# tensorboy/pytorch_Realtime_Multi-Person_Pose_Estimation

Hardware: AMD Instinct MI355X
Metric: end-to-end persons-posed FPS at 368x368 (net+pafprocess) (higher is better)
Workload: dtype fp32; 1 GPU; rtpose VGG19 368x368 batch=32 synthetic images, single MI355X, fp32 (BASELINE.json configs[1]); per-GPU batch 32, one process per GPU; global_batch=32, weights=seeded He init (no checkpoint offline), decoder_input=synthetic scene + 1e-3 * net output (blend kernel timed), humans_per_batch=163, parallelism=single GPU

## Files before the change

pytorch_realtime_multi-person_pose_estimation_amd/csrc/conv_wino7.hip:

```cpp
#include <hip/hip_runtime.h>

#include <cstdlib>

#include "conv_desc.h"
#include "launchers.h"
#include "wino_common.h"

namespace rtpose {

namespace wino7 {

using namespace winoc;

constexpr int W7_PF = 4;

template <int FM>
struct WT;
template <>
struct WT<4> {
  static constexpr int NFQ = 10, NP = 4, NSETS = 5;
  __device__ static constexpr float kPts[4] = {1.f, 2.f, 0.5f, 1.5f};
  __device__ static constexpr float kBT[10][10] = {
      {2.25f, 0.f, -12.8125f, 0.f, 17.0625f, 0.f, -7.5f, 0.f, 1.f, 0.f},
      {0.f, -2.25f, -2.25f, 10.5625f, 10.5625f, -6.5f, -6.5f, 1.f, 1.f, 0.f},
      {0.f, 2.25f, -2.25f, -10.5625f, 10.5625f, 6.5f, -6.5f, -1.f, 1.f, 0.f},
      {0.f, -1.125f, -0.5625f, 6.125f, 3.0625f, -7.f, -3.5f, 2.f, 1.f, 0.f},
      {0.f, 1.125f, -0.5625f, -6.125f, 3.0625f, 7.f, -3.5f, -2.f, 1.f, 0.f},
      {0.f, -4.5f, -9.f, 7.625f, 15.25f, -3.625f, -7.25f, 0.5f, 1.f, 0.f},
      {0.f, 4.5f, -9.f, -7.625f, 15.25f, 3.625f, -7.25f, -0.5f, 1.f, 0.f},
      {0.f, -1.5f, -1.f, 7.875f, 5.25f, -7.875f, -5.25f, 1.5f, 1.f, 0.f},
      {0.f, 1.5f, -1.f, -7.875f, 5.25f, 7.875f, -5.25f, -1.5f, 1.f, 0.f},
      {0.f, 2.25f, 0.f, -12.8125f, 0.f, 17.0625f, 0.f, -7.5f, 0.f, 1.f},
  };
};
template <>
struct WT<6> {
  static constexpr int NFQ = 12, NP = 5, NSETS = 6;
  __device__ static constexpr float kPts[5] = {1.f, 2.f, 0.5f, 1.5f, 0.666666667f};
  __device__ static constexpr float kBT[12][12] = {
      {-1.f, 0.f, 7.94444444f, 0.f, -20.3958333f, 0.f, 20.3958333f, 0.f, -7.94444444f, 0.f, 1.f, 0.f},
      {0.f, 1.f, 1.f, -6.94444444f, -6.94444444f, 13.4513889f, 13.4513889f, -6.94444444f, -6.94444444f, 1.f, 1.f, 0.f},
      {0.f, -1.f, 1.f, 6.94444444f, -6.94444444f, -13.4513889f, 13.4513889f, 6.94444444f, -6.94444444f, -1.f, 1.f, 0.f},
      {0.f, 0.5f, 0.25f, -3.84722222f, -1.92361111f, 9.23611111f, 4.61805556f, -7.88888889f, -3.94444444f, 2.f, 1.f, 0.f},
      {0.f, -0.5f, 0.25f, 3.84722222f, -1.92361111f, -9.23611111f, 4.61805556f, 7.88888889f, -3.94444444f, -2.f, 1.f, 0.f},
      {0.f, 2.f, 4.f, -7.88888889f, -15.7777778f, 9.23611111f, 18.4722222f, -3.84722222f, -7.69444444f, 0.5f, 1.f, 0.f},
      {0.f, -2.f, 4.f, 7.88888889f, -15.7777778f, -9.23611111f, 18.4722222f, 3.84722222f, -7.69444444f, -0.5f, 1.f, 0.f},
      {0.f, 0.666666667f, 0.444444444f, -5.f, -3.33333333f, 11.375f, 7.58333333f, -8.54166667f, -5.69444444f, 1.5f, 1.f, 0.f},
      {0.f, -0.666666667f, 0.444444444f, 5.f, -3.33333333f, -11.375f, 7.58333333f, 8.54166667f, -5.69444444f, -1.5f, 1.f, 0.f},
      {0.f, 1.5f, 2.25f, -8.54166667f, -12.8125f, 11.375f, 17.0625f, -5.f, -7.5f, 0.666666667f, 1.f, 0.f},
      {0.f, -1.5f, 2.25f, 8.54166667f, -12.8125f, -11.375f, 17.0625f, 5.f, -7.5f, -0.666666667f, 1.f, 0.f},
      {0.f, -1.f, 0.f, 7.94444444f, 0.f, -20.3958333f, 0.f, 20.3958333f, 0.f, -7.94444444f, 0.f, 1.f},
  };
};

template <>
struct WT<8> {
  static constexpr int NFQ = 14, NP = 6, NSETS = 7;
  __device__ static constexpr float kPts[6] = {1.f, 2.f, 0.5f, 1.5f, 0.666666667f, 1.25f};
  __device__ static constexpr float kBT[14][14] = {
      {1.5625f, 0.f, -13.4131944f, 0.f, 39.812934f, 0.f, -52.2643229f, 0.f, 32.8090278f, 0.f, -9.50694444f, 0.f, 1.f, 0.f},
      {0.f, -1.5625f, -1.5625f, 11.8506944f, 11.8506944f, -27.9622396f, -27.9622396f, 24.3020833f, 24.3020833f, -8.50694444f, -8.50694444f, 1.f, 1.f, 0.f},
      {0.f, 1.5625f, -1.5625f, -11.8506944f, 11.8506944f, 27.9622396f, -27.9622396f, -24.3020833f, 24.3020833f, 8.50694444f, -8.50694444f, -1.f, 1.f, 0.f},
      {0.f, -0.78125f, -0.390625f, 6.51128472f, 3.25564236f, -18.2786458f, -9.13932292f, 21.5625f, 10.78125f, -11.0138889f, -5.50694444f, 2.f, 1.f, 0.f},
      {0.f, 0.78125f, -0.390625f, -6.51128472f, 3.25564236f, 18.2786458f, -9.13932292f, -21.5625f, 10.78125f, 11.0138889f, -5.50694444f, -2.f, 1.f, 0.f},
      {0.f, -3.125f, -6.25f, 14.3263889f, 28.6527778f, -22.3203125f, -44.640625f, 15.2473958f, 30.4947917f, -4.62847222f, -9.25694444f, 0.5f, 1.f, 0.f},
      {0.f, 3.125f, -6.25f, -14.3263889f, 28.6527778f, 22.3203125f, -44.640625f, -15.2473958f, 30.4947917f, 4.62847222f, -9.25694444f, -0.5f, 1.f, 0.f},
      {0.f, -1.04166667f, -0.694444444f, 8.47916667f, 5.65277778f, -22.7734375f, -15.1822917f, 24.7213542f, 16.4809028f, -10.8854167f, -7.25694444f, 1.5f, 1.f, 0.f},
      {0.f, 1.04166667f, -0.694444444f, -8.47916667f, 5.65277778f, 22.7734375f, -15.1822917f, -24.7213542f, 16.4809028f, 10.8854167f, -7.25694444f, -1.5f, 1.f, 0.f},
      {0.f, -2.34375f, -3.515625f, 14.8463542f, 22.2695312f, -26.3151042f, -39.4726562f, 19.1875f, 28.78125f, -6.04166667f, -9.0625f, 0.666666667f, 1.f, 0.f},
      {0.f, 2.34375f, -3.515625f, -14.8463542f, 22.2695312f, 26.3151042f, -39.4726562f, -19.1875f, 28.78125f, 6.04166667f, -9.0625f, -0.666666667f, 1.f, 0.f},
      {0.f, -1.25f, -1.f, 9.93055556f, 7.94444444f, -25.4947917f, -20.3958333f, 25.4947917f, 20.3958333f, -9.93055556f, -7.94444444f, 1.25f, 1.f, 0.f},
      {0.f, 1.25f, -1.f, -9.93055556f, 7.94444444f, 25.4947917f, -20.3958333f, -25.4947917f, 20.3958333f, 9.93055556f, -7.94444444f, -1.25f, 1.f, 0.f},
      {0.f, 1.5625f, 0.f, -13.4131944f, 0.f, 39.812934f, 0.f, -52.2643229f, 0.f, 32.8090278f, 0.f, -9.50694444f, 0.f, 1.f},
  };
};

#define RTPOSE_W7_POINTS {0.0, 1.0, -1.0, 2.0, -2.0, 0.5, -0.5, 1.5, -1.5, 2.0 / 3.0, -2.0 / 3.0, 1.25, -1.25}

struct Group {
  const float* in;
  const float* w;
  const float* bias;
  float* out;
  int in_cstride, in_choff, in_ws, in_hs, in_lead;
  int out_cstride, out_choff, out_ws, out_hs, out_lead;
  int cout, cout_pad;
  size_t in_bytes, w_bytes;
};

struct Args {
  Group g[2];
  int N, H, W;
  int GX, T;
  int TPI;
  int cin, relu;
  int RS;
  int VB;
  int mtiles, ntiles, ncombo, xcd_remap;
  int persist;
  float* scratch;
  int* flags;
  int* err;
};

__device__ float llvm_raw_buffer_load_f32(i32x4 rsrc, int voffset, int soffset, int aux) __asm(
    "llvm.amdgcn.raw.buffer.load.f32");

constexpr int CK = 8, CG = 2;

__host__ __device__ constexpr int row_stride(int gx, int nfq) {
  int rs = nfq * CG * gx;
  while ((rs & 15) != (gx & 15)) ++rs;
  return rs;
}
__host__ __device__ constexpr int strip_rows(int gx) { return (31 + gx - 1) / gx + 1 + 6; }

template <int NI, int FM>
struct Xform {
  using T = WT<FM>;
  static constexpr int NFQ = T::NFQ, NP = T::NP, NHI = NFQ - 7;
  i32x4 rin;
  unsigned voff[NI], vhi[NI][NHI], pxb;
  int vdst[NI], fstride;
  F4 d[NI][NFQ], eo[2];

  __device__ __forceinline__ void setup(const Group& g, int W, int GX, int RS, int R0, int nrows) {
    const int tid = threadIdx.x;
    const int nitems = nrows * GX * CG;
    const long qbase = (long)g.in_lead + (long)(R0 - 3) * g.in_ws - 3;
    const size_t o0 = (size_t)qbase * g.in_cstride + g.in_choff;
    rin = make_rsrc(g.in + o0, g.in_bytes - o0 * 4);
#pragma unroll
    for (int k = 0; k < NI; ++k) {
      const int i = min((tid & 255) + k * 256, nitems - 1);
      const int r = i / (GX * CG), rem = i - r * (GX * CG);
      const int cg = rem / GX, gx = rem - cg * GX;
      voff[k] = (unsigned)((((long)r * g.in_ws + FM * gx) * g.in_cstride + cg * 4) * 4);
      vdst[k] = r * RS + cg * GX + gx;
#pragma unroll
      for (int n = 7; n < NFQ; ++n) vhi[k][n - 7] = voff[k] + (unsigned)(min(n, W + 5 - FM * gx) * g.in_cstride * 4);
    }
    pxb = (unsigned)g.in_cstride * 4;
    fstride = CG * GX;
  }
  __device__ __forceinline__ void load_piece(int chunk, int k, int n) {
    const unsigned cb = (unsigned)chunk * (CK * 4);
    d[k][n] = n < 7 ? bload(rin, voff[k], cb + n * pxb) : bload(rin, vhi[k][n < 7 ? 0 : n - 7], cb);
  }
  __device__ __forceinline__ void tgroup(float4* vw, int k, int gidx) {
    if (gidx < NP) {
      const int row = 2 * gidx + 1;
#pragma unroll
      for (int odd = 0; odd < 2; ++odd) {
        const int n0 = odd ? 1 : 2;
        F4 s = mul4(T::kBT[row][n0], d[k][n0]);
#pragma unroll
        for (int t = 1; t < NP; ++t) s = fma4(T::kBT[row][n0 + 2 * t], d[k][n0 + 2 * t], s);
        eo[odd] = s;
      }
      vw[vdst[k] + row * fstride] = to_float4(add4(eo[0], eo[1]));
      vw[vdst[k] + (row + 1) * fstride] = to_float4(sub4(eo[0], eo[1]));
    } else {
      const int f = gidx == NP ? 0 : NFQ - 1, n0 = gidx == NP ? 0 : 1;
      F4 s = mul4(T::kBT[f][n0], d[k][n0]);
#pragma unroll
      for (int t = 1; t < NP + 1; ++t) s = fma4(T::kBT[f][n0 + 2 * t], d[k][n0 + 2 * t], s);
      vw[vdst[k] + f * fstride] = to_float4(s);
    }
  }
};

template <int NI, int GXT, int FM, int FS>
__device__ __forceinline__ void wino7_segment(const Args& A, float4* V4, const int mt, const int c, const int cb,
                                              const int ce, const int nch, const int slot) {
  using T = WT<FM>;
  constexpr int NFQ = T::NFQ, NP = T::NP;
  constexpr int NFW = NFQ / FS;
  static_assert(NFW % 2 == 0, "frequency pairs");
  constexpr int NSETS = FS == 2 ? 7 : (FM == 6 && NI == 2) ? 3 : T::NSETS;
  constexpr int NPS = 7 * NFW / 2;
  constexpr int PF = FS == 2 ? NSETS - 1 : (W7_PF < NSETS ? W7_PF : NSETS - 1);
  static_assert(NPS % NSETS == 0, "B register sets must rotate in step with the chunk");
  const int tid = threadIdx.x;
  const int lane = tid & 63;
  const int wv = __builtin_amdgcn_readfirstlane(tid >> 6);
  const int wn = FS == 2 ? (wv & 3) : wv, fh = FS == 2 ? (wv >> 2) : 0;
  const bool xf = wv < 4;
  auto my_group = [&](int gi) { return true || (gi & 1) == fh; };
  const int l31 = lane & 31, kh = lane >> 5;
  const int nt = c % A.ntiles, grp = c / A.ntiles;
  const Group g = grp ? A.g[1] : A.g[0];
  const int GX = GXT ? GXT : A.GX;
  const int RS = GXT ? row_stride(GXT, NFQ) : A.RS;
  const int VB = GXT ? strip_rows(GXT) * row_stride(GXT, NFQ) : A.VB;
  const int PI = A.H * GX;

  int t0, tlim;
  if (A.TPI) {
    const int n = mt / A.TPI;
    t0 = n * PI + (mt - n * A.TPI) * 32;
    tlim = (n + 1) * PI;
  } else {
    t0 = mt * 32;
    tlim = A.T;
  }
  int R0, nrows;
  {
    const int n0 = t0 / PI, y0 = (t0 - n0 * PI) / GX;
    const int t1 = min(t0 + 31, tlim - 1);
    const int n1 = t1 / PI, y1 = (t1 - n1 * PI) / GX;
    R0 = n0 * g.in_hs + y0;
    nrows = n1 * g.in_hs + y1 - R0 + 7;
  }
  Xform<NI, FM> X;
  X.setup(g, A.W, GX, RS, R0, nrows);
  const i32x4 rw = make_rsrc(g.w, g.w_bytes);
  auto load_piece = [&](int chunk, int k, int n) { X.load_piece(chunk, k, n); };
  auto tgroup = [&](float4* vw, int k, int gidx) { X.tgroup(vw, k, gidx); };

  int abase;
  {
    const int t = min(t0 + l31, tlim - 1);
    const int n = t / PI, r = t - n * PI;
    const int y = r / GX, gx = r - y * GX;
    abase = (n * g.in_hs + y - R0) * RS + kh * GX + gx + (fh * NFW) * CG * GX;
  }
  const int ncol = nt * 128 + wn * 32 + l31;
  floatx16 acc[NFW];
  float* sp = A.scratch + ((size_t)(slot * 4 + wn) * (NFQ * 16) + (size_t)fh * NFW * 16) * 64 + lane;
  if (FM == 8) {
    if (cb > 0) {
      if (tid == 0) {
        unsigned spins = 0;
        while (__hip_atomic_load(A.flags + slot, __ATOMIC_ACQUIRE, __HIP_MEMORY_SCOPE_AGENT) != 1) {
          __builtin_amdgcn_s_sleep(8);
          if (++spins > (1u << 22)) {
            __hip_atomic_fetch_or(A.err, 1, __ATOMIC_RELAXED, __HIP_MEMORY_SCOPE_AGENT);
            break;
          }
        }
      }
      __syncthreads();
      __builtin_amdgcn_fence(__ATOMIC_ACQUIRE, "agent");
    }
    const i32x4 rs = make_rsrc(sp - lane, cb > 0 ? (size_t)NFW * 16 * 64 * sizeof(float) : 0);
    const float b0 = g.bias[ncol];
#pragma unroll
    for (int f = 0; f < NFW; ++f)
#pragma unroll
      for (int r = 0; r < 16; ++r) {
        const float v = llvm_raw_buffer_load_f32(rs, lane * 4, (f * 16 + r) * 256, 0);
        acc[f][r] = (f == 1 && cb == 0) ? b0 : v;
      }
    if (cb > 0) {
      __syncthreads();
      if (tid == 0) __hip_atomic_store(A.flags + slot, 0, __ATOMIC_RELAXED, __HIP_MEMORY_SCOPE_AGENT);
    }
  } else if (cb == 0) {
#pragma unroll
    for (int f = 0; f < NFW; ++f)
#pragma unroll
      for (int r = 0; r < 16; ++r) acc[f][r] = 0.f;
    if (fh == 0) {
      const float b0 = g.bias[ncol];
#pragma unroll
      for (int r = 0; r < 16; ++r) acc[1][r] = b0;
    }
  } else {
    if (tid == 0) {
      unsigned spins = 0;
      while (__hip_atomic_load(A.flags + slot, __ATOMIC_ACQUIRE, __HIP_MEMORY_SCOPE_AGENT) != 1) {
        __builtin_amdgcn_s_sleep(8);
        if (++spins > (1u << 22)) {
          __hip_atomic_fetch_or(A.err, 1, __ATOMIC_RELAXED, __HIP_MEMORY_SCOPE_AGENT);
          break;
        }
      }
    }
    __syncthreads();
    __builtin_amdgcn_fence(__ATOMIC_ACQUIRE, "agent");
#pragma unroll
    for (int f = 0; f < NFW; ++f)
#pragma unroll
      for (int r = 0; r < 16; ++r) acc[f][r] = sp[(f * 16 + r) * 64];
    __syncthreads();
    if (tid == 0) __hip_atomic_store(A.flags + slot, 0, __ATOMIC_RELAXED, __HIP_MEMORY_SCOPE_AGENT);
  }
  const unsigned boff = (unsigned)((kh * g.cout_pad + ncol) * 16);
  const unsigned fstep = (unsigned)(CG * g.cout_pad * 16);
  unsigned wso = ((unsigned)cb * (7 * NFQ) + (unsigned)(fh * NFW)) * fstep;
  int bl = 0;
  auto bnext = [&](int& cnt) {
    wso += fstep;
    if (++cnt == NFW) {
      cnt = 0;
      if (FS > 1) wso += (unsigned)(NFQ - NFW) * fstep;
    }
  };
  float4 bs[NSETS][2];

  if (xf) {
#pragma unroll
    for (int k = 0; k < NI; ++k)
#pragma unroll
      for (int n = 0; n < NFQ; ++n) load_piece(cb, k, n);
#pragma unroll
    for (int k = 0; k < NI; ++k)
#pragma unroll
      for (int gi = 0; gi < NP + 2; ++gi)
        tgroup(V4, k, gi);
    const int c1 = min(cb + 1, ce - 1);
#pragma unroll
    for (int k = 0; k < NI; ++k)
#pragma unroll
      for (int n = 0; n < NFQ; ++n) load_piece(c1, k, n);
  }
#pragma unroll
  for (int s = 0; s < PF; ++s) {
    bs[s][0] = bload_f4(rw, boff, wso);
    bnext(bl);
    bs[s][1] = bload_f4(rw, boff, wso);
    bnext(bl);
  }
  __syncthreads();

#define RTPOSE_PIN()             \
  asm volatile("" ::: "memory"); \
  __builtin_amdgcn_sched_barrier(0)
  constexpr int NG = (NP + 2) * NI, GSTR = (NI == 1 && FS == 1) ? 2 : 1, LS = NG * GSTR;
  constexpr int LPS = 1, LSTEPS = (NFQ * NI + LPS - 1) / LPS;
  static_assert(LS + LSTEPS <= NPS, "transform work does not fit the steps of a chunk");
  float4 a[2][2];
  for (int chunk = cb; chunk < ce; ++chunk) {
    const float4* va = V4 + ((chunk - cb) & 1) * VB + abase;
    float4* vw = V4 + ((chunk - cb + 1) & 1) * VB;
    const int c2 = min(chunk + 2, ce - 1);
    a[0][0] = va[0];
    a[0][1] = va[CG * GX];
#pragma unroll
    for (int ps = 0; ps < NPS; ++ps) {
      const int fp = ps % (NFW / 2);
#pragma unroll
      for (int j = 0; j < 4; ++j) {
        {
          const float4 a0 = a[ps & 1][0], a1 = a[ps & 1][1], b0 = bs[ps % NSETS][0], b1 = bs[ps % NSETS][1];
          const float a0v[4] = {a0.x, a0.y, a0.z, a0.w}, a1v[4] = {a1.x, a1.y, a1.z, a1.w};
          const float b0v[4] = {b0.x, b0.y, b0.z, b0.w}, b1v[4] = {b1.x, b1.y, b1.z, b1.w};
          acc[2 * fp] = __builtin_amdgcn_mfma_f32_32x32x2f32(a0v[j], b0v[j], acc[2 * fp], 0, 0, 0);
          acc[2 * fp + 1] = __builtin_amdgcn_mfma_f32_32x32x2f32(a1v[j], b1v[j], acc[2 * fp + 1], 0, 0, 0);
        }
        RTPOSE_PIN();
        if (j < 2) {
          if (ps + 1 < NPS) {
            const int kyn = (ps + 1) / (NFW / 2), fn = 2 * ((ps + 1) % (NFW / 2)) + j;
            a[(ps + 1) & 1][j] = va[kyn * RS + fn * CG * GX];
          }
        } else {
          bs[(ps + PF) % NSETS][j - 2] = bload_f4(rw, boff, wso);
          bnext(bl);
        }
        if (j == 3 && xf) {
          if (ps % GSTR == 0 && ps / GSTR < NG) {
            if (xf && my_group((ps / GSTR) % (NP + 2))) tgroup(vw, (ps / GSTR) / (NP + 2), (ps / GSTR) % (NP + 2));
          } else if (ps >= LS && ps < LS + LSTEPS) {
#pragma unroll
            for (int q = 0; q < LPS; ++q) {
              const int l = LPS * (ps - LS) + q;
              if (l < NFQ * NI) load_piece(c2, l / NFQ, l % NFQ);
            }
          }
        }
        RTPOSE_PIN();
      }
    }
    __syncthreads();
  }
#undef RTPOSE_PIN

  if (ce < nch) {
#pragma unroll
    for (int f = 0; f < NFW; ++f)
#pragma unroll
      for (int r = 0; r < 16; ++r) sp[(f * 16 + r) * 64] = acc[f][r];
    __builtin_amdgcn_fence(__ATOMIC_RELEASE, "agent");
    __syncthreads();
    if (tid == 0) __hip_atomic_store(A.flags + slot, 1, __ATOMIC_RELEASE, __HIP_MEMORY_SCOPE_AGENT);
    return;
  }

  const bool col_ok = ncol < g.cout;
  float* out_base = g.out + g.out_choff + ncol;
  constexpr int R0E = 16 / FS;
  float* E = reinterpret_cast<float*>(V4);
  if (FS == 2) {
    float* ew = E + (size_t)((wn * 2 + fh) * NFW * 8) * 64 + lane;
#pragma unroll
    for (int f = 0; f < NFW; ++f)
#pragma unroll
      for (int rl = 0; rl < 8; ++rl) ew[(f * 8 + rl) * 64] = fh ? acc[f][rl] : acc[f][8 + rl];
    __syncthreads();
  }
  const float* er = E + (size_t)((wn * 2 + (1 - fh)) * NFW * 8) * 64 + lane;
  int tcur = t0 + (FS == 2 ? 16 * fh : 0) + 4 * kh;
  int sn = tcur / PI, sy, sx;
  {
    const int r = tcur - sn * PI;
    sy = r / GX;
    sx = r - sy * GX;
  }
#pragma unroll
  for (int rr = 0; rr < R0E; ++rr) {
    const int r = rr;
    float m[NFQ];
    if (FS == 2) {
#pragma unroll
      for (int f = 0; f < NFW; ++f) {
        const float own = fh ? acc[f][8 + rr] : acc[f][rr];
        const float oth = er[(f * 8 + rr) * 64];
        m[f] = fh ? oth : own;
        m[NFW + f] = fh ? own : oth;
      }
    } else {
#pragma unroll
      for (int f = 0; f < NFQ; ++f) m[f] = acc[f % NFW][rr];
    }
    float S[NP], D[NP];
#pragma unroll
    for (int p = 0; p < NP; ++p) {
      S[p] = m[2 * p + 1] + m[2 * p + 2];
      D[p] = m[2 * p + 1] - m[2 * p + 2];
    }
    float y[FM];
#pragma unroll
    for (int i = 0; i < FM; ++i) {
      float v = (i & 1) ? D[0] : S[0];
      float pw[NP];
#pragma unroll
      for (int p = 1; p < NP; ++p) {
        pw[p] = 1.f;
        for (int e = 0; e < i; ++e) pw[p] *= T::kPts[p];
        v = __builtin_fmaf(pw[p], (i & 1) ? D[p] : S[p], v);
      }
      if (i == 0) v += m[0];
      if (i == FM - 1) v += m[NFQ - 1];
      y[i] = v;
    }
    if (col_ok && tcur < tlim) {
      const size_t q = (size_t)g.out_lead + (size_t)(sn * g.out_hs + sy) * g.out_ws + FM * sx;
#pragma unroll
      for (int i = 0; i < FM; ++i) {
        const float v = A.relu ? fmaxf(y[i], 0.f) : y[i];
        if (FM * sx + i < A.W) out_base[(q + i) * g.out_cstride] = v;
      }
    }
    const int dstep = (r & 3) == 3 ? 5 : 1;
    tcur += dstep;
    sx += dstep;
    while (sx >= GX) {
      sx -= GX;
      if (++sy >= A.H) {
        sy = 0;
        ++sn;
      }
    }
  }
  if (FS == 2) __syncthreads();
}

template <int NI, int GXT, int FM, int FS>
__global__ __launch_bounds__(256 * FS, 1) void wino7_f32(const Args A) {
  extern __shared__ __attribute__((aligned(16))) float4 V4[];
  const int nch = A.cin / CK;
  long u0, u1;
  if (A.persist) {
    const long U = (long)A.mtiles * A.ncombo * nch, P = gridDim.x, p = blockIdx.x;
    u0 = p * U / P;
    u1 = (p + 1) * U / P;
  } else {
    const int bi = blockIdx.x;
    int mt, c;
    if (A.xcd_remap) {
      const int xcd = bi & 7, j = bi >> 3;
      c = j % A.ncombo;
      mt = (j / A.ncombo) * 8 + xcd;
    } else {
      mt = bi % A.mtiles;
      c = bi / A.mtiles;
    }
    if (mt >= A.mtiles) return;
    u0 = ((long)mt * A.ncombo + c) * nch;
    u1 = u0 + nch;
  }
  const int tf = (int)(u0 / nch), cbf = (int)(u0 - (long)tf * nch);
  const int tl = (int)((u1 - 1) / nch), cel = (int)(u1 - (long)tl * nch);
  const int nseg = tl - tf + 1;
  for (int i = 0; i < nseg; ++i) {
    int tile, cb = 0, ce = nch;
    const bool head_first = cel < nch && nseg > 1, tail_last = cbf > 0;
    if (head_first && i == 0) {
      tile = tl;
      ce = cel;
    } else if (tail_last && i == nseg - 1) {
      tile = tf;
      cb = cbf;
      if (tf == tl) ce = cel;
    } else {
      tile = tf + i - (head_first ? 1 : 0) + (tail_last ? 1 : 0);
      if (tile == tl) ce = cel;
    }
    const int mt = tile / A.ncombo, c = tile - mt * A.ncombo;
    wino7_segment<NI, GXT, FM, FS>(A, V4, mt, c, cb, ce, nch, cb > 0 ? (int)blockIdx.x - 1 : (int)blockIdx.x);
  }
}

template <int NI>
__global__ __launch_bounds__(256, 1) void wino7s_f32(const Args A) {
  constexpr int FM = 6;
  using T = WT<FM>;
  constexpr int NFQ = T::NFQ, NP = T::NP, FW = NFQ / 4;
  constexpr int NSETS = 7, PF = 3;
  extern __shared__ __attribute__((aligned(16))) float4 V4[];
  const int tid = threadIdx.x;
  const int lane = tid & 63;
  const int wv = __builtin_amdgcn_readfirstlane(tid >> 6);
  const int l31 = lane & 31, kh = lane >> 5;
  const int bi = blockIdx.x;
  const int c = bi % A.ncombo, mt = bi / A.ncombo;
  const int nt = c % A.ntiles, grp = c / A.ntiles;
  const Group g = grp ? A.g[1] : A.g[0];
  const int GX = A.GX, RS = A.RS, VB = A.VB;
  const int PI = A.H * GX;
  int t0, tlim;
  if (A.TPI) {
    const int n = mt / A.TPI;
    t0 = n * PI + (mt - n * A.TPI) * 32;
    tlim = (n + 1) * PI;
  } else {
    t0 = mt * 32;
    tlim = A.T;
  }
  int R0, nrows;
  {
    const int n0 = t0 / PI, y0 = (t0 - n0 * PI) / GX;
    const int t1 = min(t0 + 31, tlim - 1);
    const int n1 = t1 / PI, y1 = (t1 - n1 * PI) / GX;
    R0 = n0 * g.in_hs + y0;
    nrows = n1 * g.in_hs + y1 - R0 + 7;
  }
  Xform<NI, FM> X;
  X.setup(g, A.W, GX, RS, R0, nrows);
  const i32x4 rw = make_rsrc(g.w, g.w_bytes);

  int abase;
  {
    const int t = min(t0 + l31, tlim - 1);
    const int n = t / PI, r = t - n * PI;
    const int y = r / GX, gx = r - y * GX;
    abase = (n * g.in_hs + y - R0) * RS + kh * GX + gx + (wv * FW) * CG * GX;
  }
  const int ncol = nt * 32 + l31;
  floatx16 acc[FW];
#pragma unroll
  for (int f = 0; f < FW; ++f)
#pragma unroll
    for (int r = 0; r < 16; ++r) acc[f][r] = 0.f;
  if (wv == 0) {
    const float b0 = g.bias[ncol];
#pragma unroll
    for (int r = 0; r < 16; ++r) acc[1][r] = b0;
  }
  const unsigned boff = (unsigned)((kh * g.cout_pad + ncol) * 16);
  const unsigned fstep = (unsigned)(CG * g.cout_pad * 16);
  const unsigned kstep = (unsigned)NFQ * fstep;
  const int nchunks = A.cin / CK;
  unsigned wso = (unsigned)(wv * FW) * fstep;
  const unsigned wso_max = wso + (unsigned)(nchunks * 7 - 1) * kstep;
  float4 bs[NSETS][FW];

#pragma unroll
  for (int k = 0; k < NI; ++k)
#pragma unroll
    for (int n = 0; n < NFQ; ++n) X.load_piece(0, k, n);
#pragma unroll
  for (int k = 0; k < NI; ++k)
#pragma unroll
    for (int gi = 0; gi < NP + 2; ++gi) X.tgroup(V4, k, gi);
  {
    const int c1 = min(1, nchunks - 1);
#pragma unroll
    for (int k = 0; k < NI; ++k)
#pragma unroll
      for (int n = 0; n < NFQ; ++n) X.load_piece(c1, k, n);
  }
#pragma unroll
  for (int s = 0; s < PF; ++s) {
#pragma unroll
    for (int f = 0; f < FW; ++f) bs[s][f] = bload_f4(rw, boff, wso + f * fstep);
    wso = min(wso + kstep, wso_max);
  }
  __syncthreads();

#define RTPOSE_PIN()             \
  asm volatile("" ::: "memory"); \
  __builtin_amdgcn_sched_barrier(0)
  constexpr int NG = (NP + 2) * NI;
  static_assert(NG <= 8 * NI && NFQ <= 12 && NI <= 2, "transform work does not fit the slots of a chunk");
  float4 a[2][FW];
  for (int chunk = 0; chunk < nchunks; ++chunk) {
    const float4* va = V4 + (chunk & 1) * VB + abase;
    float4* vw = V4 + ((chunk + 1) & 1) * VB;
    const int c2 = min(chunk + 2, nchunks - 1);
#pragma unroll
    for (int f = 0; f < FW; ++f) a[0][f] = va[f * CG * GX];
#pragma unroll
    for (int ky = 0; ky < 7; ++ky) {
#pragma unroll
      for (int j = 0; j < 4; ++j) {
#pragma unroll
        for (int f = 0; f < FW; ++f) {
          const float4 av = a[ky & 1][f], bv = bs[ky % NSETS][f];
          const float avv[4] = {av.x, av.y, av.z, av.w}, bvv[4] = {bv.x, bv.y, bv.z, bv.w};
          acc[f] = __builtin_amdgcn_mfma_f32_32x32x2f32(avv[j], bvv[j], acc[f], 0, 0, 0);
        }
        RTPOSE_PIN();
        if (j == 0) {
          if (ky + 1 < 7) {
#pragma unroll
            for (int f = 0; f < FW; ++f) a[(ky + 1) & 1][f] = va[(ky + 1) * RS + f * CG * GX];
          }
        } else if (j == 1) {
#pragma unroll
          for (int f = 0; f < FW; ++f) bs[(ky + PF) % NSETS][f] = bload_f4(rw, boff, wso + f * fstep);
          wso = min(wso + kstep, wso_max);
        } else {
          const int slot = 2 * ky + (j - 2);
#pragma unroll
          for (int q = 0; q < NI; ++q) {
            if (ky < 4) {
              const int gq = slot * NI + q;
              if (gq < NG) X.tgroup(vw, gq / (NP + 2), gq % (NP + 2));
            } else {
#pragma unroll
              for (int h = 0; h < 2; ++h) {
                const int l = ((slot - 8) * NI + q) * 2 + h;
                if (l < NFQ * NI) X.load_piece(c2, l / NFQ, l % NFQ);
              }
            }
          }
        }
        RTPOSE_PIN();
      }
    }
    __syncthreads();
  }
#undef RTPOSE_PIN

  float* E = reinterpret_cast<float*>(V4);
#pragma unroll
  for (int f = 0; f < FW; ++f)
#pragma unroll
    for (int r = 0; r < 16; ++r) E[((wv * FW + f) * 16 + r) * 64 + lane] = acc[f][r];
  __syncthreads();
  const bool col_ok = ncol < g.cout;
  float* out_base = g.out + g.out_choff + ncol;
  int tcur = t0 + 8 * wv + 4 * kh;
  int sn = tcur / PI, sy, sx;
  {
    const int r = tcur - sn * PI;
    sy = r / GX;
    sx = r - sy * GX;
  }
#pragma unroll
  for (int rr = 0; rr < 4; ++rr) {
    const int r = 4 * wv + rr;
    float m[NFQ];
#pragma unroll
    for (int f = 0; f < NFQ; ++f) m[f] = E[(f * 16 + r) * 64 + lane];
    float S[NP], D[NP];
#pragma unroll
    for (int p = 0; p < NP; ++p) {
      S[p] = m[2 * p + 1] + m[2 * p + 2];
      D[p] = m[2 * p + 1] - m[2 * p + 2];
    }
    float y[FM];
#pragma unroll
    for (int i = 0; i < FM; ++i) {
      float v = (i & 1) ? D[0] : S[0];
      float pw[NP];
#pragma unroll
      for (int p = 1; p < NP; ++p) {
        pw[p] = 1.f;
        for (int e = 0; e < i; ++e) pw[p] *= T::kPts[p];
        v = __builtin_fmaf(pw[p], (i & 1) ? D[p] : S[p], v);
      }
      if (i == 0) v += m[0];
      if (i == FM - 1) v += m[NFQ - 1];
      y[i] = v;
    }
    if (col_ok && tcur < tlim) {
      const size_t q = (size_t)g.out_lead + (size_t)(sn * g.out_hs + sy) * g.out_ws + FM * sx;
#pragma unroll
      for (int i = 0; i < FM; ++i) {
        const float v = A.relu ? fmaxf(y[i], 0.f) : y[i];
        if (FM * sx + i < A.W) out_base[(q + i) * g.out_cstride] = v;
      }
    }
    ++tcur;
    if (++sx >= GX) {
      sx = 0;
      if (++sy >= A.H) {
        sy = 0;
        ++sn;
      }
    }
  }
}

__global__ void pack_wino7_kernel(const float* __restrict__ w, const float* __restrict__ bias, int cout,
                                  int cin_src, const int32_t* __restrict__ cin_map, int cin_packed, int coutp,
                                  int nfq, float* __restrict__ wp, float* __restrict__ bp) {
  const size_t total = (size_t)7 * nfq * cin_packed * coutp;
  const size_t i = (size_t)blockIdx.x * blockDim.x + threadIdx.x;
  if (i < (size_t)coutp) bp[i] = (i < (size_t)cout && bias) ? bias[i] : 0.f;
  if (i >= total) return;
  const int e = i & 3;
  size_t r = i >> 2;
  const int n = r % coutp;
  r /= coutp;
  const int cg = r % CG;
  r /= CG;
  const int f = r % nfq;
  r /= nfq;
  const int ky = r % 7;
  const int chunk = r / 7;
  const int c = chunk * CK + cg * 4 + e;
  const int src = cin_map ? cin_map[c] : (c < cin_src ? c : -1);
  float v = 0.f;
  if (n < cout && src >= 0 && src < cin_src) {
    const float* gw = w + (((size_t)n * cin_src + src) * 7 + ky) * 7;
    if (f == nfq - 1) {
      v = gw[6];
    } else {
      const double pts[13] = RTPOSE_W7_POINTS;
      double nf = 1.0;
      for (int l = 0; l < nfq - 1; ++l)
        if (l != f) nf *= pts[f] - pts[l];
      double s = 0.0, pw = 1.0;
      for (int kx = 0; kx < 7; ++kx) {
        s += pw * (double)gw[kx];
        pw *= pts[f];
      }
      v = (float)(s / nf);
    }
  }
  wp[i] = v;
}

int wino7_default_fm() {
  static int fm = 0;
  if (!fm) {
    const char* e = getenv("RTPOSE_WINOGRAD7_M");
    fm = (e && e[0] == '4') ? 4 : 6;
  }
  return fm;
}
static int resolve_fm(int fm) { return fm == 0 ? wino7_default_fm() : fm; }

struct Plan {
  int fm, nfq, gx, rs, nrows, ni, tpi, mtiles;
  long T;
  size_t lds;
};

static int make_plan(int N, int H, int W, int hs, int fm, Plan* p) {
  p->fm = fm;
  p->nfq = p->fm + 6;
  p->gx = ceil_div(W, p->fm);
  p->rs = row_stride(p->gx, p->nfq);
  p->T = (long)N * H * p->gx;
  if (p->T > 0x7fffffffL) return -1;
  const int pi = H * p->gx;
  p->tpi = pi >= 256 ? ceil_div(pi, 32) : 0;
  int nrows = 0;
  if (p->tpi) {
    nrows = strip_rows(p->gx) < H + 6 ? strip_rows(p->gx) : H + 6;
    p->mtiles = N * p->tpi;
  } else {
    for (long t0 = 0; t0 < p->T; t0 += 32) {
      const long t1 = t0 + 31 < p->T - 1 ? t0 + 31 : p->T - 1;
      const int n0 = (int)(t0 / pi), y0 = (int)((t0 - (long)n0 * pi) / p->gx);
      const int n1 = (int)(t1 / pi), y1 = (int)((t1 - (long)n1 * pi) / p->gx);
      const int rows = (n1 * hs + y1) - (n0 * hs + y0) + 7;
      if (rows > nrows) nrows = rows;
    }
    p->mtiles = (int)((p->T + 31) / 32);
  }
  p->nrows = nrows;
  p->ni = ceil_div(nrows * p->gx * CG, 256);
  p->lds = (size_t)2 * nrows * p->rs * 16;
  return 0;
}

template <int NI, int GXT, int FM, int FS = 1>
static int launch_inst(const Args& a, dim3 grid, size_t lds, hipStream_t s) {
  const size_t ex = FS == 2 ? (size_t)4 * 2 * (FM + 6) / 2 * 8 * 64 * sizeof(float) : 0;
  return launch_kernel<wino7_f32<NI, GXT, FM, FS>>(grid, dim3(256 * FS), lds > ex ? lds : ex, 160 * 1024, s, a);
}

template <int NI>
static int launch_small(const Args& a, dim3 grid, size_t lds, hipStream_t s) {
  return launch_kernel<wino7s_f32<NI>>(grid, dim3(256), lds, 160 * 1024, s, a);
}

template <int FM>
__device__ float bt_abs_row_sum(int f) {
  float b = 0.f;
  for (int n = 0; n < WT<FM>::NFQ; ++n) b += fabsf(WT<FM>::kBT[f][n]);
  return b;
}

__global__ void wino_amp_kernel(const float* __restrict__ w, int cout, int cin, int k, int fm, float* __restrict__ amp) {
  __shared__ float red[17][256];
  const int o = blockIdx.x, tid = threadIdx.x;
  float sf[16], den = 0.f;
#pragma unroll
  for (int f = 0; f < 16; ++f) sf[f] = 0.f;
  const int nfq = fm + 6;
  const double pts[13] = RTPOSE_W7_POINTS;
  __shared__ double s_nf[14];
  if (k == 7 && tid < nfq - 1) {
    double nf = 1.0;
    for (int l = 0; l < nfq - 1; ++l)
      if (l != tid) nf *= pts[tid] - pts[l];
    s_nf[tid] = nf;
  }
  __syncthreads();
  for (int c = tid; c < cin; c += 256) {
    const float* gw = w + ((size_t)o * cin + c) * k * k;
    if (k == 3) {
      float u[4][3];
      for (int x = 0; x < 3; ++x) {
        const float g0 = gw[x], g1 = gw[3 + x], g2 = gw[6 + x];
        u[0][x] = g0;
        u[1][x] = 0.5f * (g0 + g1 + g2);
        u[2][x] = 0.5f * (g0 - g1 + g2);
        u[3][x] = g2;
        den += fabsf(g0) + fabsf(g1) + fabsf(g2);
      }
      for (int fy = 0; fy < 4; ++fy) {
        sf[fy * 4 + 0] += fabsf(u[fy][0]);
        sf[fy * 4 + 1] += fabsf(0.5f * (u[fy][0] + u[fy][1] + u[fy][2]));
        sf[fy * 4 + 2] += fabsf(0.5f * (u[fy][0] - u[fy][1] + u[fy][2]));
        sf[fy * 4 + 3] += fabsf(u[fy][2]);
      }
    } else {
      for (int ky = 0; ky < 7; ++ky) {
        const float* row = gw + ky * 7;
        for (int kx = 0; kx < 7; ++kx) den += fabsf(row[kx]);
        for (int f = 0; f < nfq; ++f) {
          double v;
          if (f == nfq - 1) {
            v = row[6];
          } else {
            const double nf = s_nf[f];
            double sacc = 0.0, pw = 1.0;
            for (int kx = 0; kx < 7; ++kx) {
              sacc += pw * (double)row[kx];
              pw *= pts[f];
            }
            v = sacc / nf;
          }
          sf[f] += fabsf((float)v);
        }
      }
    }
  }
#pragma unroll
  for (int f = 0; f < 16; ++f) red[f][tid] = sf[f];
  red[16][tid] = den;
  __syncthreads();
  for (int st = 128; st > 0; st >>= 1) {
    if (tid < st)
      for (int f = 0; f < 17; ++f) red[f][tid] += red[f][tid + st];
    __syncthreads();
  }
  if (tid == 0) {
    float num = 0.f;
    if (k == 3) {
      const float a[2][4] = {{1.f, 1.f, 1.f, 0.f}, {0.f, 1.f, 1.f, 1.f}};
      for (int i = 0; i < 2; ++i)
        for (int j = 0; j < 2; ++j) {
          float v = 0.f;
          for (int fy = 0; fy < 4; ++fy)
            for (int fx = 0; fx < 4; ++fx) v += a[i][fy] * a[j][fx] * 4.f * red[fy * 4 + fx][0];
          num = fmaxf(num, v);
        }
    } else {
      const float pabs[14] = {0.f, 1.f, 1.f, 2.f, 2.f, 0.5f, 0.5f, 1.5f, 1.5f, 0.666666667f, 0.666666667f, 1.25f, 1.25f, 0.f};
      for (int i = 0; i < fm; ++i) {
        float v = 0.f;
        for (int f = 0; f < nfq; ++f) {
          const float b = fm == 4 ? bt_abs_row_sum<4>(f) : fm == 6 ? bt_abs_row_sum<6>(f) : bt_abs_row_sum<8>(f);
          float ai;
          if (f == 0) ai = i == 0 ? 1.f : 0.f;
          else if (f == nfq - 1) ai = i == fm - 1 ? 1.f : 0.f;
          else {
            ai = 1.f;
            for (int e = 0; e < i; ++e) ai *= pabs[f];
          }
          v += ai * b * red[f][0];
        }
        num = fmaxf(num, v);
      }
    }
    const float r = red[16][0] > 0.f ? num / red[16][0] : 0.f;
    atomicMax(reinterpret_cast<int*>(amp), __float_as_int(r));
  }
}

}

int wino7_default_fm() { return wino7::wino7_default_fm(); }

static size_t wino7_scratch_flag_bytes(int blocks) { return round_up((size_t)(blocks + 2) * sizeof(int), 256); }
int* conv2d_wino7_scratch_err(void* scratch, int blocks) { return static_cast<int*>(scratch) + blocks + 1; }
size_t conv2d_wino7_scratch_bytes(int blocks, int fm) {
  const int nfq = (fm == 8 ? 8 : 6) + 6;
  return wino7_scratch_flag_bytes(blocks) + (size_t)blocks * (4 * nfq * 16 * 64) * sizeof(float);
}

int conv2d_wino7_fits(int cin, int cout, int N, int H, int W, int hs, int fm) {
  fm = wino7::resolve_fm(fm);
  if ((fm != 4 && fm != 6 && fm != 8) || cin <= 0 || cin % wino7::CK || cout_pad(cout) % 128 || N <= 0 || H <= 0 || W <= 0) return 0;
  wino7::Plan p;
  if (wino7::make_plan(N, H, W, hs, fm, &p)) return 0;
  return p.ni <= 2 && p.lds <= 156 * 1024;
}

double conv2d_wino7_issued_flops(int cin, int cout, int N, int H, int W, int hs, int fm) {
  fm = wino7::resolve_fm(fm);
  wino7::Plan p;
  if (wino7::make_plan(N, H, W, hs, fm, &p)) return 0.0;
  return 2.0 * p.mtiles * 32.0 * 7.0 * p.nfq * (double)cin * cout_pad(cout);
}

int conv2d_wino7_launch(const rtpose_conv_desc* d, int ngroups, int N, int H, int W, int fm, void* scratch,
                        size_t scratch_bytes, hipStream_t s) {
  using namespace wino7;
  fm = resolve_fm(fm);
  const ConvSpec spec = {"conv2d_winograd (7x7)", 4, 1, false, false, false, true};
  if (int rc = check_conv_features(d, ngroups, spec)) return rc;
  const rtpose_conv_desc& d0 = d[0];
  if (d0.k != 7 || d0.pool || !conv2d_wino7_fits(d0.cin, d0.cout, N, H, W, d0.lin.hs, fm))
    return fail(RTPOSE_E_INVAL, "%s: no F(%d,7) instance for cin %d cout %d at %d x %d x %d", spec.who, fm, d0.cin,
                d0.cout, N, H, W);
  if (int rc = check_conv_layouts(d, ngroups, N, H, W, spec)) return rc;
  Args a;
  memset(&a, 0, sizeof(a));
  for (int i = 0; i < ngroups; ++i) {
    const rtpose_conv_desc& di = d[i];
    Group& g = a.g[i];
    fill_group(g, di);
    g.in_bytes = rtpose_layout_pixels(&di.lin, N, H, W) * (size_t)di.lin.cstride * sizeof(float);
    g.w_bytes = packed_weight_floats_wino7(di.cout, di.cin, fm) * sizeof(float);
  }
  Plan p;
  make_plan(N, H, W, d0.lin.hs, fm, &p);
  a.N = N;
  a.H = H;
  a.W = W;
  a.GX = p.gx;
  a.T = (int)p.T;
  a.cin = d0.cin;
  a.relu = d0.relu;
  a.RS = p.rs;
  a.VB = p.nrows * p.rs;
  a.TPI = p.tpi;
  a.mtiles = p.mtiles;
  a.ntiles = cout_pad(d0.cout) / 128;
  a.ncombo = a.ntiles * ngroups;
  long ids;
  if (int rc = grid_ids(a.mtiles, a.ncombo, a.xcd_remap, ids, spec.who)) return rc;
  {
    const int n_cu = device_cu_count();
    const long tiles = (long)a.mtiles * a.ncombo;
    if (tiles >= n_cu && tiles % n_cu != 0 && scratch && scratch_bytes >= conv2d_wino7_scratch_bytes(n_cu, fm)) {
      if ((uintptr_t)scratch & 255) return fail(RTPOSE_E_INVAL, "conv2d_winograd: scratch must be 256-byte aligned");
      a.flags = static_cast<int*>(scratch);
      a.err = a.flags + n_cu + 1;
      a.scratch = reinterpret_cast<float*>(static_cast<char*>(scratch) + wino7_scratch_flag_bytes(n_cu));
      RTPOSE_HIP_CHECK(hipMemsetAsync(a.flags, 0, (size_t)(n_cu + 1) * sizeof(int), s));
      a.persist = 1;
      ids = n_cu;
    }
  }
  const dim3 grid((unsigned)ids, 1, 1);
  if (p.fm == 6 && !a.persist && (long)a.mtiles * a.ncombo * 2 <= device_cu_count()) {
    Args b = a;
    b.ntiles = cout_pad(d0.cout) / 32;
    b.ncombo = b.ntiles * ngroups;
    const dim3 gs((unsigned)((long)b.mtiles * b.ncombo), 1, 1);
    const size_t lds_s = p.lds > (size_t)12 * 16 * 64 * 4 ? p.lds : (size_t)12 * 16 * 64 * 4;
    return p.ni == 1 ? launch_small<1>(b, gs, lds_s, s) : launch_small<2>(b, gs, lds_s, s);
  }
  if (p.fm == 6) {
    if (p.gx == 8 && p.tpi && p.ni == 1 && p.nrows == strip_rows(8))
      return launch_inst<1, 8, 6, 2>(a, grid, (size_t)2 * strip_rows(8) * row_stride(8, 12) * 16, s);
    if (p.ni == 1) return launch_inst<1, 0, 6, 2>(a, grid, p.lds, s);
    return launch_inst<2, 0, 6>(a, grid, p.lds, s);
  }
  if (p.fm == 8) {
    if (p.gx == 6 && p.tpi && p.ni == 1 && p.nrows == strip_rows(6))
      return launch_inst<1, 6, 8>(a, grid, (size_t)2 * strip_rows(6) * row_stride(6, 14) * 16, s);
    if (p.ni == 1) return launch_inst<1, 0, 8>(a, grid, p.lds, s);
    return launch_inst<2, 0, 8>(a, grid, p.lds, s);
  }
  if (p.gx == 12 && p.tpi && p.ni == 1 && p.nrows == strip_rows(12))
    return launch_inst<1, 12, 4>(a, grid, (size_t)2 * strip_rows(12) * row_stride(12, 10) * 16, s);
  if (p.ni == 1) return launch_inst<1, 0, 4>(a, grid, p.lds, s);
  return launch_inst<2, 0, 4>(a, grid, p.lds, s);
}

int pack_weights_wino7_launch(const float* w, const float* bias, int cout, int cin_src, const int32_t* cin_map,
                              int cin_packed, int fm, float* wp, float* bp, hipStream_t s) {
  fm = wino7::resolve_fm(fm);
  if (fm != 4 && fm != 6 && fm != 8) return fail(RTPOSE_E_INVAL, "pack_winograd: F(m,7) exists for m = 4, 6 and 8");
  if (cin_packed % wino7::CK || cin_packed <= 0 || (cin_packed < cin_src && !cin_map))
    return fail(RTPOSE_E_INVAL, "pack_winograd: cin_packed must be a multiple of 8 and >= cin_src");
  const int coutp = cout_pad(cout);
  const int nfq = fm + 6;
  const size_t total = (size_t)7 * nfq * cin_packed * coutp;
  const int threads = 256;
  const unsigned blocks = (unsigned)((total + threads - 1) / threads);
  hipLaunchKernelGGL(wino7::pack_wino7_kernel, dim3(blocks), dim3(threads), 0, s, w, bias, cout, cin_src, cin_map,
                     cin_packed, coutp, nfq, wp, bp);
  RTPOSE_HIP_CHECK(hipGetLastError());
  return 0;
}

size_t packed_weight_floats_wino7(int cout, int cin, int fm) {
  return (size_t)(7 * (wino7::resolve_fm(fm) + 6) * cin + 96) * cout_pad(cout);
}

int wino_amplification_launch(const float* w, int cout, int cin, int k, int fm, float* amp, hipStream_t s) {
  if (k == 7) fm = wino7::resolve_fm(fm);
  if (!w || !amp || cout <= 0 || cin <= 0 || !(k == 3 || (k == 7 && (fm == 4 || fm == 6 || fm == 8))))
    return fail(RTPOSE_E_INVAL, "winograd_amplification: k must be 3, or 7 with m = 4, 6 or 8");
  RTPOSE_HIP_CHECK(hipMemsetAsync(amp, 0, sizeof(float), s));
  hipLaunchKernelGGL(wino7::wino_amp_kernel, dim3((unsigned)cout), dim3(256), 0, s, w, cout, cin, k, k == 7 ? fm : 0, amp);
  RTPOSE_HIP_CHECK(hipGetLastError());
  return 0;
}

}
```

Before: 1448 images/s.

## Pack Winograd 7x7 tiles across image boundaries and gate persistent mode

The F(m,7) Winograd planner may now choose flat tiling, where 32-tile blocks span image boundaries, when per-image tiling would waste partially filled tiles and the row footprint still fits the same number of loader items and the LDS limit. The row scan only covers one period of the tile pattern. The GX-specialised instances now accept any strip up to a padded row count (inst_rows), so they also handle flat plans. The persistent-scheduling path for F(6,7) single-item plans now runs only when the tail wave wastes more than 15% of slots. The intent is fewer tiles, less wasted work at image edges, and no persistent-mode overhead when its benefit is small. In exchange, the specialised kernels use more LDS and may need more rows per strip.

```diff
diff --git a/pytorch_realtime_multi-person_pose_estimation_amd/csrc/conv_wino7.hip b/pytorch_realtime_multi-person_pose_estimation_amd/csrc/conv_wino7.hip
--- a/pytorch_realtime_multi-person_pose_estimation_amd/csrc/conv_wino7.hip
+++ b/pytorch_realtime_multi-person_pose_estimation_amd/csrc/conv_wino7.hip
@@ -114,6 +114,7 @@
   return rs;
 }
 __host__ __device__ constexpr int strip_rows(int gx) { return (31 + gx - 1) / gx + 1 + 6; }
+__host__ __device__ constexpr int inst_rows(int gx) { return (32 % gx ? strip_rows(gx) : 32 / gx + 6) + 3; }
 
 template <int NI, int FM>
 struct Xform {
@@ -192,7 +193,7 @@
   const Group g = grp ? A.g[1] : A.g[0];
   const int GX = GXT ? GXT : A.GX;
   const int RS = GXT ? row_stride(GXT, NFQ) : A.RS;
-  const int VB = GXT ? strip_rows(GXT) * row_stride(GXT, NFQ) : A.VB;
+  const int VB = GXT ? inst_rows(GXT) * row_stride(GXT, NFQ) : A.VB;
   const int PI = A.H * GX;
 
   int t0, tlim;
@@ -772,6 +773,8 @@
   size_t lds;
 };
 
+constexpr size_t kMaxLds = 156 * 1024;
+
 static int make_plan(int N, int H, int W, int hs, int fm, Plan* p) {
   p->fm = fm;
   p->nfq = p->fm + 6;
@@ -780,24 +783,28 @@
   p->T = (long)N * H * p->gx;
   if (p->T > 0x7fffffffL) return -1;
   const int pi = H * p->gx;
-  p->tpi = pi >= 256 ? ceil_div(pi, 32) : 0;
-  int nrows = 0;
-  if (p->tpi) {
-    nrows = strip_rows(p->gx) < H + 6 ? strip_rows(p->gx) : H + 6;
-    p->mtiles = N * p->tpi;
-  } else {
-    for (long t0 = 0; t0 < p->T; t0 += 32) {
-      const long t1 = t0 + 31 < p->T - 1 ? t0 + 31 : p->T - 1;
-      const int n0 = (int)(t0 / pi), y0 = (int)((t0 - (long)n0 * pi) / p->gx);
-      const int n1 = (int)(t1 / pi), y1 = (int)((t1 - (long)n1 * pi) / p->gx);
-      const int rows = (n1 * hs + y1) - (n0 * hs + y0) + 7;
-      if (rows > nrows) nrows = rows;
-    }
-    p->mtiles = (int)((p->T + 31) / 32);
-  }
-  p->nrows = nrows;
-  p->ni = ceil_div(nrows * p->gx * CG, 256);
-  p->lds = (size_t)2 * nrows * p->rs * 16;
+  int gcd = 32;
+  while (pi % gcd) gcd >>= 1;
+  const long period = (long)pi / gcd * 32;
+  int flat_rows = 0;
+  for (long t0 = 0; t0 < p->T && t0 < period; t0 += 32) {
+    const long t1 = t0 + 31 < p->T - 1 ? t0 + 31 : p->T - 1;
+    const int n0 = (int)(t0 / pi), y0 = (int)((t0 - (long)n0 * pi) / p->gx);
+    const int n1 = (int)(t1 / pi), y1 = (int)((t1 - (long)n1 * pi) / p->gx);
+    const int rows = (n1 * hs + y1) - (n0 * hs + y0) + 7;
+    if (rows > flat_rows) flat_rows = rows;
+  }
+  const long flat_tiles = (p->T + 31) / 32;
+  const int tpi = ceil_div(pi, 32);
+  const int img_rows = strip_rows(p->gx) < H + 6 ? strip_rows(p->gx) : H + 6;
+  const bool flat = pi < 256 || (flat_tiles < (long)N * tpi &&
+                                 ceil_div(flat_rows * p->gx * CG, 256) == ceil_div(img_rows * p->gx * CG, 256) &&
+                                 (size_t)2 * flat_rows * p->rs * 16 <= kMaxLds);
+  p->tpi = flat ? 0 : tpi;
+  p->mtiles = flat ? (int)flat_tiles : N * tpi;
+  p->nrows = flat ? flat_rows : img_rows;
+  p->ni = ceil_div(p->nrows * p->gx * CG, 256);
+  p->lds = (size_t)2 * p->nrows * p->rs * 16;
   return 0;
 }
 
@@ -934,7 +941,7 @@
   if ((fm != 4 && fm != 6 && fm != 8) || cin <= 0 || cin % wino7::CK || cout_pad(cout) % 128 || N <= 0 || H <= 0 || W <= 0) return 0;
   wino7::Plan p;
   if (wino7::make_plan(N, H, W, hs, fm, &p)) return 0;
-  return p.ni <= 2 && p.lds <= 156 * 1024;
+  return p.ni <= 2 && p.lds <= wino7::kMaxLds;
 }
 
 double conv2d_wino7_issued_flops(int cin, int cout, int N, int H, int W, int hs, int fm) {
@@ -984,7 +991,9 @@
   {
     const int n_cu = device_cu_count();
     const long tiles = (long)a.mtiles * a.ncombo;
-    if (tiles >= n_cu && tiles % n_cu != 0 && scratch && scratch_bytes >= conv2d_wino7_scratch_bytes(n_cu, fm)) {
+    const long slots = (long)ceil_div(tiles, n_cu) * n_cu;
+    const bool pays = !(p.fm == 6 && p.ni == 1) || (slots - tiles) * 100 > 15 * slots;
+    if (tiles >= n_cu && tiles % n_cu != 0 && pays && scratch && scratch_bytes >= conv2d_wino7_scratch_bytes(n_cu, fm)) {
       if ((uintptr_t)scratch & 255) return fail(RTPOSE_E_INVAL, "conv2d_winograd: scratch must be 256-byte aligned");
       a.flags = static_cast<int*>(scratch);
       a.err = a.flags + n_cu + 1;
@@ -1004,19 +1013,19 @@
     return p.ni == 1 ? launch_small<1>(b, gs, lds_s, s) : launch_small<2>(b, gs, lds_s, s);
   }
   if (p.fm == 6) {
-    if (p.gx == 8 && p.tpi && p.ni == 1 && p.nrows == strip_rows(8))
-      return launch_inst<1, 8, 6, 2>(a, grid, (size_t)2 * strip_rows(8) * row_stride(8, 12) * 16, s);
+    if (p.gx == 8 && p.ni == 1 && p.nrows <= inst_rows(8))
+      return launch_inst<1, 8, 6, 2>(a, grid, (size_t)2 * inst_rows(8) * row_stride(8, 12) * 16, s);
     if (p.ni == 1) return launch_inst<1, 0, 6, 2>(a, grid, p.lds, s);
     return launch_inst<2, 0, 6>(a, grid, p.lds, s);
   }
   if (p.fm == 8) {
-    if (p.gx == 6 && p.tpi && p.ni == 1 && p.nrows == strip_rows(6))
-      return launch_inst<1, 6, 8>(a, grid, (size_t)2 * strip_rows(6) * row_stride(6, 14) * 16, s);
+    if (p.gx == 6 && p.ni == 1 && p.nrows <= inst_rows(6))
+      return launch_inst<1, 6, 8>(a, grid, (size_t)2 * inst_rows(6) * row_stride(6, 14) * 16, s);
     if (p.ni == 1) return launch_inst<1, 0, 8>(a, grid, p.lds, s);
     return launch_inst<2, 0, 8>(a, grid, p.lds, s);
   }
-  if (p.gx == 12 && p.tpi && p.ni == 1 && p.nrows == strip_rows(12))
-    return launch_inst<1, 12, 4>(a, grid, (size_t)2 * strip_rows(12) * row_stride(12, 10) * 16, s);
+  if (p.gx == 12 && p.ni == 1 && p.nrows <= inst_rows(12))
+    return launch_inst<1, 12, 4>(a, grid, (size_t)2 * inst_rows(12) * row_stride(12, 10) * 16, s);
   if (p.ni == 1) return launch_inst<1, 0, 4>(a, grid, p.lds, s);
   return launch_inst<2, 0, 4>(a, grid, p.lds, s);
 }
```

Result: no change. 1442 images/s (-0.4%).
